# Exidekat/TransformerUpscaler

Hardware: AMD Instinct MI355X
Metric: images/sec, FastTransformer 2x 720p->1080p inference (higher is better)
Workload: dtype bf16

## Files before the change

transformerupscaler_amd/csrc/conv3x3_c64.hip:

```cpp
#include "conv_pingpong.h"
#include <stdlib.h>

namespace {

constexpr int TH = 8, TW = 32;
constexpr int in_tile_bytes(int ks) { return (TH + ks - 1) * (TW + ks - 1) * 128; }

enum { OUT_NHWC_BF16 = 0, OUT_PLANAR_F32 = 1 };

template <int CT, int OUT_MODE, int KS>
__global__ __launch_bounds__(256, (CT <= 4 && KS == 3) ? 2 : 1) void conv3x3_c64_kernel(
    const bf16_t* __restrict__ x, const bf16_t* __restrict__ wp, const float* __restrict__ bias,
    const bf16_t* __restrict__ add, const bf16_t* __restrict__ mask,
    void* __restrict__ out, int H, int W, int ntiles, int r, int cout_valid, int relu,
    int tilesX, int tilesY, int in_r)
{
    constexpr int PADK = KS / 2, HALO_W = TW + KS - 1, HALO_H = TH + KS - 1, NPIX_HALO = HALO_H * HALO_W;
    constexpr int NTAPS = KS * KS;
    extern __shared__ __attribute__((aligned(16))) char smem[];
    char* in_lds = smem;
    char* w_lds = smem + in_tile_bytes(KS);
    constexpr int WROWS = CT * 16;
    constexpr int WSLAB = WROWS * 128;
    constexpr int WCH = WROWS * 8;
    constexpr int WREGS = (WCH + 255) / 256;

    const int tid = threadIdx.x, lane = tid & 63, wave = tid >> 6;
    const int g = lane >> 4, p = lane & 15;
    int bid = blockIdx.x;
    const int tx = bid % tilesX; bid /= tilesX;
    const int ty = bid % tilesY;
    const int b = bid / tilesY;
    const int ty0 = ty * TH, tx0 = tx * TW;

    const int nci = in_r * in_r;
    const int Hin = H * in_r, Win = W * in_r;
    const bf16_t* xb = x + (size_t)b * Hin * Win * 64;
    constexpr int NSI = (NPIX_HALO * 8 + 255) / 256;
    auto stage_input = [&](int ci) {
        const int si = ci / in_r, sj = ci - si * in_r;
        u32x4 v[NSI];
        auto pos = [&](int idx, int& q, int& c, size_t& off) -> bool {
            q = idx >> 3; c = idx & 7;
            const int yy = q / HALO_W, xx = q - yy * HALO_W;
            const int iy = ty0 - PADK + yy, ix = tx0 - PADK + xx;
            const bool ok = idx < NPIX_HALO * 8 && iy >= 0 && iy < H && ix >= 0 && ix < W;
            off = ok ? ((size_t)(iy * in_r + si) * Win + (ix * in_r + sj)) * 64 + c * 8 : 0;
            return ok;
        };
#pragma unroll
        for (int k = 0; k < NSI; ++k) {
            int q, c; size_t off;
            pos(tid + k * 256, q, c, off);
            v[k] = *reinterpret_cast<const u32x4*>(xb + off);
        }
#pragma unroll
        for (int k = 0; k < NSI; ++k) {
            const int idx = tid + k * 256;
            int q, c; size_t off;
            const bool ok = pos(idx, q, c, off);
            if (idx < NPIX_HALO * 8) *reinterpret_cast<u32x4*>(in_lds + swz128(q, c)) = ok ? v[k] : u32x4{0u, 0u, 0u, 0u};
        }
    };
    stage_input(0);

    u32x4 wreg[WREGS];
    auto wload = [&](int it) {
#pragma unroll
        for (int u = 0; u < WREGS; ++u) {
            const int idx = tid + u * 256;
            if (idx < WCH) wreg[u] = *reinterpret_cast<const u32x4*>(wp + (size_t)it * WROWS * 64 + idx * 8);
        }
    };
    auto wstore = [&](int buf) {
#pragma unroll
        for (int u = 0; u < WREGS; ++u) {
            const int idx = tid + u * 256;
            if (idx < WCH) *reinterpret_cast<u32x4*>(w_lds + buf * WSLAB + swz128(idx >> 3, idx & 7)) = wreg[u];
        }
    };

    int qb[4];
#pragma unroll
    for (int pg = 0; pg < 4; ++pg) qb[pg] = (2 * wave + (pg >> 1)) * HALO_W + (pg & 1) * 16 + p;

    f32x4 acc[4][CT], bv[CT];
    const int total = ntiles * nci * NTAPS;
    wload(0);
    wstore(0);
    __syncthreads();

    for (int it = 0; it < total; ++it) {
        const int tap = it % NTAPS, chunk_it = it / NTAPS;
        const int ci = chunk_it % nci, nt = chunk_it / nci;
        const int buf = it & 1;
        if (tap == 0 && it > 0 && nci > 1) {
            stage_input(ci);
            __syncthreads();
        }
        if (it + 1 < total) wload(it + 1);
        if (tap == 0 && ci == 0) {
#pragma unroll
            for (int pg = 0; pg < 4; ++pg)
#pragma unroll
                for (int ct = 0; ct < CT; ++ct) acc[pg][ct] = f32x4{0.f, 0.f, 0.f, 0.f};
#pragma unroll
            for (int ct = 0; ct < CT; ++ct) {
                bv[ct] = f32x4{0.f, 0.f, 0.f, 0.f};
                if (bias) {
                    if constexpr (OUT_MODE == OUT_NHWC_BF16) bv[ct] = *reinterpret_cast<const f32x4*>(bias + nt * 64 + g * 16 + ct * 4);
                    else {
#pragma unroll
                        for (int e = 0; e < 4; ++e) { const int co = 16 * ct + 4 * g + e; bv[ct][e] = co < cout_valid ? bias[co] : 0.f; }
                    }
                }
            }
        }
        const int dy = tap / KS, dx = tap - dy * KS;
        const int qoff = dy * HALO_W + dx;
        const char* wb = w_lds + buf * WSLAB;
#pragma unroll
        for (int kh = 0; kh < 2; ++kh) {
            const int chunk = kh * 4 + g;
            bf16x8 pf[4], wf[CT];
#pragma unroll
            for (int pg = 0; pg < 4; ++pg)
                pf[pg] = *reinterpret_cast<const bf16x8*>(in_lds + swz128(qb[pg] + qoff, chunk));
#pragma unroll
            for (int ct = 0; ct < CT; ++ct)
                wf[ct] = *reinterpret_cast<const bf16x8*>(wb + swz128(ct * 16 + p, chunk));
#pragma unroll
            for (int pg = 0; pg < 4; ++pg)
#pragma unroll
                for (int ct = 0; ct < CT; ++ct) acc[pg][ct] = mfma16x16x32(wf[ct], pf[pg], acc[pg][ct]);
        }
        if (it + 1 < total) wstore(buf ^ 1);
        __syncthreads();

        if (tap == NTAPS - 1 && ci == nci - 1) {
#pragma unroll
            for (int pg = 0; pg < 4; ++pg) {
                const int oy = ty0 + 2 * wave + (pg >> 1);
                const int ox = tx0 + (pg & 1) * 16 + p;
                if (oy >= H || ox >= W) continue;
                if constexpr (OUT_MODE == OUT_NHWC_BF16) {
                    const int si = nt / r, sj = nt - si * r;
                    const int Hr = H * r, Wr = W * r;
                    bf16_t* o = reinterpret_cast<bf16_t*>(out) +
                                (((size_t)b * Hr + (oy * r + si)) * Wr + (ox * r + sj)) * 64 + g * 16;
                    uint32_t pk[8];
                    const size_t eoff = (((size_t)b * Hr + (oy * r + si)) * Wr + (ox * r + sj)) * 64 + g * 16;
                    uint32_t aw[8], mw[8];
                    if (add) {
                        const u32x4 a0 = *reinterpret_cast<const u32x4*>(add + eoff), a1 = *reinterpret_cast<const u32x4*>(add + eoff + 8);
#pragma unroll
                        for (int q = 0; q < 4; ++q) { aw[q] = a0[q]; aw[4 + q] = a1[q]; }
                    }
                    if (mask) {
                        const u32x4 m0 = *reinterpret_cast<const u32x4*>(mask + eoff), m1 = *reinterpret_cast<const u32x4*>(mask + eoff + 8);
#pragma unroll
                        for (int q = 0; q < 4; ++q) { mw[q] = m0[q]; mw[4 + q] = m1[q]; }
                    }
#pragma unroll
                    for (int ct = 0; ct < CT; ++ct) {
                        float v[4];
#pragma unroll
                        for (int e = 0; e < 4; ++e) {
                            v[e] = acc[pg][ct][e];
                            v[e] += bv[ct][e];
                            if (relu) v[e] = fmaxf(v[e], 0.f);
                            const int wi = (ct * 4 + e) >> 1;
                            if (add) v[e] += __builtin_bit_cast(float, (e & 1) ? (aw[wi] & 0xffff0000u) : (aw[wi] << 16));
                            if (mask) {
                                const float mv = __builtin_bit_cast(float, (e & 1) ? (mw[wi] & 0xffff0000u) : (mw[wi] << 16));
                                if (!(mv > 0.f)) v[e] = 0.f;
                            }
                        }
                        pk[ct * 2 + 0] = pack_bf16x2(v[0], v[1]);
                        pk[ct * 2 + 1] = pack_bf16x2(v[2], v[3]);
                    }
                    if constexpr (CT == 4) {
                        *reinterpret_cast<u32x4*>(o) = u32x4{pk[0], pk[1], pk[2], pk[3]};
                        *reinterpret_cast<u32x4*>(o + 8) = u32x4{pk[4], pk[5], pk[6], pk[7]};
                    }
                } else {
                    float* o = reinterpret_cast<float*>(out);
                    const int rr = r * r, cimg = cout_valid / rr, Hr = H * r, Wr = W * r;
#pragma unroll
                    for (int ct = 0; ct < CT; ++ct)
#pragma unroll
                        for (int e = 0; e < 4; ++e) {
                            const int co = 16 * ct + 4 * g + e;
                            if (co < cout_valid) {
                                float v = acc[pg][ct][e];
                                v += bv[ct][e];
                                if (relu) v = fmaxf(v, 0.f);
                                const int c = co / rr, sp = co - c * rr;
                                const int si = sp / r, sj = sp - si * r;
                                o[(((size_t)b * cimg + c) * Hr + (oy * r + si)) * Wr + (ox * r + sj)] = v;
                            }
                        }
                }
            }
        }
    }
}



__device__ unsigned long long tup_conv_stamps[2][16][5];

template <int CT, int OUT_MODE, int KS>
__global__ __launch_bounds__(512, 2) void conv_c64_persistent_kernel(
    const bf16_t* __restrict__ x, const bf16_t* __restrict__ wp, const float* __restrict__ bias,
    const bf16_t* __restrict__ add, const bf16_t* __restrict__ mask,
    void* __restrict__ out, int B, int H, int W, int ntiles, int r, int cout_valid, int relu,
    int tilesX, int tilesY, int stamps)
{
    constexpr int PADK = KS / 2, HALO_W = TW + KS - 1, HALO_H = TH + KS - 1, NPIX_HALO = HALO_H * HALO_W;
    constexpr int NTAPS = KS * KS;
    constexpr int IN_BYTES = NPIX_HALO * 128;
    constexpr int WROWS = CT * 16, WSLAB = WROWS * 128;
    extern __shared__ __attribute__((aligned(16))) char smem[];
    char* w_lds = smem;
    char* in_lds = smem + NTAPS * WSLAB;

    const int grp = __builtin_amdgcn_readfirstlane((int)(threadIdx.x >> 8));
    const int tid = threadIdx.x & 255, lane = tid & 63, wave = tid >> 6;
    const int g = lane >> 4, p = lane & 15;
    const int total_tiles = tilesX * tilesY * B;
    char* my_in = in_lds + grp * IN_BYTES;

    const HaloDma<HALO_H, HALO_W, PADK> dma(W, tid);
    auto prefetch_tile = [&](const TC& c) { dma.prefetch(x, c.b, c.ty * TH, c.tx * TW, H, W, my_in, tup_zero_line); };

    uint32_t poff[NTAPS][2];
    pixel_frag_offsets<KS, HALO_W>(poff, my_in, wave, g, p);
    const uint32_t wbase0 = weight_frag_base(w_lds, g, p);

    f32x4 acc[4][CT];
    float* bias_lds = reinterpret_cast<float*>(in_lds + 2 * IN_BYTES);
    const uint32_t bias_addr = lds_addr(bias_lds) + (uint32_t)(g * CT * 16);

    auto store_tile = [&](const TC& c, int nt) {
        const int tx = c.tx, ty = c.ty, b = c.b;
#pragma unroll
        for (int pg = 0; pg < 4; ++pg) {
            const int oy = ty * TH + 2 * wave + (pg >> 1);
            const int ox = tx * TW + (pg & 1) * 16 + p;
            const bool ok = oy < H && ox < W;
            if constexpr (OUT_MODE == OUT_NHWC_BF16) {
                const int si = nt / r, sj = nt - si * r;
                const int Hr = H * r, Wr = W * r;
                const size_t eoff = (((size_t)b * Hr + (oy * r + si)) * Wr + (ox * r + sj)) * 64 + g * 16;
                uint32_t pk[8], aw[8], mw[8];
                if (add && ok) {
                    const u32x4 a0 = *reinterpret_cast<const u32x4*>(add + eoff), a1 = *reinterpret_cast<const u32x4*>(add + eoff + 8);
#pragma unroll
                    for (int q = 0; q < 4; ++q) { aw[q] = a0[q]; aw[4 + q] = a1[q]; }
                }
                if (mask && ok) {
                    const u32x4 m0 = *reinterpret_cast<const u32x4*>(mask + eoff), m1 = *reinterpret_cast<const u32x4*>(mask + eoff + 8);
#pragma unroll
                    for (int q = 0; q < 4; ++q) { mw[q] = m0[q]; mw[4 + q] = m1[q]; }
                }
                if (!add && !mask) {
                    typedef short s16x2 __attribute__((ext_vector_type(2)));
#pragma unroll
                    for (int ct = 0; ct < CT; ++ct) {
                        pk[ct * 2 + 0] = pack_bf16x2(acc[pg][ct][0], acc[pg][ct][1]);
                        pk[ct * 2 + 1] = pack_bf16x2(acc[pg][ct][2], acc[pg][ct][3]);
                    }
                    if (relu) {
#pragma unroll
                        for (int q = 0; q < 2 * CT; ++q)
                            pk[q] = __builtin_bit_cast(uint32_t, __builtin_elementwise_max(__builtin_bit_cast(s16x2, pk[q]), s16x2{0, 0}));
                    }
                } else
#pragma unroll
                for (int ct = 0; ct < CT; ++ct) {
                    float v[4];
#pragma unroll
                    for (int e = 0; e < 4; ++e) {
                        v[e] = acc[pg][ct][e];
                        if (relu) v[e] = fmaxf(v[e], 0.f);
                        const int wi = (ct * 4 + e) >> 1;
                        if (add && ok) v[e] += __builtin_bit_cast(float, (e & 1) ? (aw[wi] & 0xffff0000u) : (aw[wi] << 16));
                        if (mask && ok) {
                            const float mv = __builtin_bit_cast(float, (e & 1) ? (mw[wi] & 0xffff0000u) : (mw[wi] << 16));
                            if (!(mv > 0.f)) v[e] = 0.f;
                        }
                    }
                    pk[ct * 2 + 0] = pack_bf16x2(v[0], v[1]);
                    pk[ct * 2 + 1] = pack_bf16x2(v[2], v[3]);
                }
                if constexpr (CT == 4) {
                    bf16_t* o = ok ? reinterpret_cast<bf16_t*>(out) + eoff : reinterpret_cast<bf16_t*>(tup_store_sink) + lane * 16;
                    *reinterpret_cast<u32x4*>(o) = u32x4{pk[0], pk[1], pk[2], pk[3]};
                    *reinterpret_cast<u32x4*>(o + 8) = u32x4{pk[4], pk[5], pk[6], pk[7]};
                }
            } else {
                if (!ok) continue;
                float* o = reinterpret_cast<float*>(out);
                const int rr = r * r, cimg = cout_valid / rr, Hr = H * r, Wr = W * r;
                if (CT == 1 && r == 2) {
                    if (g < cimg) {
                        float v[4];
#pragma unroll
                        for (int e = 0; e < 4; ++e) v[e] = relu ? fmaxf(acc[pg][0][e], 0.f) : acc[pg][0][e];
                        float* base = o + (((size_t)b * cimg + g) * Hr + oy * 2) * Wr + ox * 2;
                        *reinterpret_cast<f32x2*>(base) = f32x2{v[0], v[1]};
                        *reinterpret_cast<f32x2*>(base + Wr) = f32x2{v[2], v[3]};
                    }
                    continue;
                }
#pragma unroll
                for (int ct = 0; ct < CT; ++ct)
#pragma unroll
                    for (int e = 0; e < 4; ++e) {
                        const int co = 16 * ct + 4 * g + e;
                        if (co < cout_valid) {
                            float v = acc[pg][ct][e];
                            if (relu) v = fmaxf(v, 0.f);
                            const int c = co / rr, sp = co - c * rr;
                            const int si = sp / r, sj = sp - si * r;
                            o[(((size_t)b * cimg + c) * Hr + (oy * r + si)) * Wr + (ox * r + sj)] = v;
                        }
                    }
            }
        }
    };

    const TileWalk walk(total_tiles, tilesX, tilesY, grp, !(stamps & 2));
    const int my_count = walk.my_count, nphases = walk.nphases;
    const TC c_first = walk.first;

    for (int nt = 0; nt < ntiles; ++nt) {
        stage_weights<CT, NTAPS>(w_lds, wp + (size_t)nt * NTAPS * WROWS * 64);
        stage_bias<CT, OUT_MODE != OUT_NHWC_BF16>(bias_lds, bias, nt, cout_valid);
        if (grp == 0 && my_count > 0) prefetch_tile(c_first);
        __syncthreads();
        TC c_done = c_first, c_next = c_first;
        if (grp == 0) walk.advance(c_next);

        const bool st_on = (stamps & 1) && blockIdx.x == 100 && (threadIdx.x & 255) == 0 && nt == 0;
        auto stamp = [&](int ph, int i) { if (st_on && ph < 16) tup_conv_stamps[grp][ph][i] = __builtin_amdgcn_s_memtime(); };
        for (int ph = 0; ph < nphases; ++ph) {
            const int k = ph >> 1;
            stamp(ph, 0);
            if ((ph & 1) == grp) {
                if (k < my_count && !(stamps & 16)) k_loop<CT, NTAPS>(acc, poff, wbase0, bias_addr);
                stamp(ph, 1);
            } else {
                const int done = grp == 0 ? k : k - 1;
                const int nxt = done + 1;
                if (nxt < my_count && !(stamps & 8)) prefetch_tile(c_next);
                stamp(ph, 1);
                if (done >= 0 && done < my_count && !(stamps & 4)) {
                    store_tile(c_done, nt);
                    stamp(ph, 2);
                    if constexpr (OUT_MODE == OUT_NHWC_BF16 && CT == 4) asm volatile("s_waitcnt vmcnt(8)" ::: "memory");
                    else asm volatile("s_waitcnt vmcnt(0)" ::: "memory");
                } else {
                    asm volatile("s_waitcnt vmcnt(0)" ::: "memory");
                }
                c_done = c_next;
                walk.advance(c_next);
            }
            asm volatile("s_waitcnt lgkmcnt(0)" ::: "memory");
            stamp(ph, 3);
            __builtin_amdgcn_s_barrier();
            stamp(ph, 4);
        }
        asm volatile("s_waitcnt vmcnt(0)" ::: "memory");
        __syncthreads();
    }
}

template <int CT, int OUT_MODE, int KS>
int launch_persistent(const void* x, const void* wp, const float* bias, const void* add, const void* mask, void* out,
                      int B, int H, int W, int ntiles, int r, int cout_valid, int relu, hipStream_t s)
{
    constexpr int NPIX_HALO = (TH + KS - 1) * (TW + KS - 1);
    constexpr size_t lds = (size_t)KS * KS * CT * 16 * 128 + 2 * (size_t)NPIX_HALO * 128 + 256;
    static_assert(lds <= 163840, "LDS budget");
    TUP_SET_DYN_LDS((conv_c64_persistent_kernel<CT, OUT_MODE, KS>), lds);
    const int tilesX = (W + TW - 1) / TW, tilesY = (H + TH - 1) / TH;
    const long long nt = (long long)tilesX * tilesY * B;
    if (nt > 0x7fffffffLL) return (int)hipErrorInvalidValue;
    const int grid = (int)(nt < 256 ? nt : 256);
#ifdef TUP_DIAG
    static const int conv_stamps_on = (getenv("TUP_CONV_STAMPS") ? 1 : 0) | (getenv("TUP_CONV_NO_XCD_BANDS") ? 2 : 0) |
                                      (getenv("TUP_CONV_ABLATE") ? (atoi(getenv("TUP_CONV_ABLATE")) & 28) : 0);
#else
    constexpr int conv_stamps_on = 0;
#endif
    conv_c64_persistent_kernel<CT, OUT_MODE, KS><<<dim3(grid), dim3(512), lds, s>>>(
        (const bf16_t*)x, (const bf16_t*)wp, bias, (const bf16_t*)add, (const bf16_t*)mask, out, B, H, W, ntiles, r,
        cout_valid, relu, tilesX, tilesY, conv_stamps_on);
    TUP_CHECK_LAUNCH();
    return 0;
}

constexpr int R5_TW = 28, R5_HW = 32, R5_HH = TH + 4, R5_NPIX = R5_HH * R5_HW, R5_IN_BYTES = R5_NPIX * 128;
constexpr int R5_W_BYTES = 5 * 64 * 128;

__global__ __launch_bounds__(512, 2) void bra_rows_persistent_kernel(
    const bf16_t* __restrict__ x, const bf16_t* __restrict__ wp, const float* __restrict__ bias,
    float* __restrict__ out, int B, int H, int W, int relu, int tilesX, int tilesY, int ablate)
{
    extern __shared__ __attribute__((aligned(16))) char smem[];
    char* w_lds = smem;
    char* in_lds = smem + R5_W_BYTES;
    const int grp = __builtin_amdgcn_readfirstlane((int)(threadIdx.x >> 8));
    const int tid = threadIdx.x & 255, lane = tid & 63, wave = tid >> 6;
    const int g = lane >> 4, p = lane & 15;
    const int total_tiles = tilesX * tilesY * B;
    char* my_in = in_lds + grp * R5_IN_BYTES;

    using Dma = HaloDma<R5_HH, R5_HW, 2>;
    static_assert(!Dma::LAST_PARTIAL && Dma::NPIECE == 12, "12 whole DMA pieces");
    const Dma dma(W, tid);
    auto prefetch_tile = [&](const TC& c) { dma.prefetch(x, c.b, c.ty * TH, c.tx * R5_TW, H, W, my_in, tup_zero_line); };

    for (int idx = threadIdx.x; idx < 5 * 64 * 8; idx += 512) {
        const int row = idx >> 3, c = idx & 7;
        const int dy = row >> 6, t = (row >> 4) & 3, r16 = row & 15;
        const int gg = r16 >> 2, sl = t * 4 + (r16 & 3);
        u32x4 v = u32x4{0u, 0u, 0u, 0u};
        if (sl < 15) {
            const int ch = sl / 5, dx = sl - ch * 5;
            v = *reinterpret_cast<const u32x4*>(wp + ((size_t)((dy * 5 + dx) * 16 + ch * 4 + gg)) * 64 + c * 8);
        }
        *reinterpret_cast<u32x4*>(w_lds + swz128(row, c)) = v;
    }
    float bch[3];
#pragma unroll
    for (int ch = 0; ch < 3; ++ch) bch[ch] = bias ? bias[ch * 4 + g] : 0.f;

    const uint32_t pbase = lds_addr(my_in) + (uint32_t)(2 * wave * R5_HW * 128) + (uint32_t)swz128(p, g);
    const uint32_t wbase = lds_addr(w_lds) + (uint32_t)swz128(p, g);

    f32x4 acc[2][2][4];
    auto compute_tile = [&]() {
        constexpr int NSTEPS = 10;
        bf16x8 pf[3][4], wf[3][4];
        auto load_frag = [&](int step, int slot, int j) {
            const int dy = step >> 1;
            if (j < 4) {
                const int off = ((j >> 1) + dy) * (R5_HW * 128) + (j & 1) * 2048;
                pf[slot][j] = (step & 1) ? lds_read_b128_asm_off_x64(pbase, off) : lds_read_b128_asm_off(pbase, off);
            } else {
                const int off = dy * 8192 + (j - 4) * 2048;
                wf[slot][j - 4] = (step & 1) ? lds_read_b128_asm_off_x64(wbase, off) : lds_read_b128_asm_off(wbase, off);
            }
        };
#pragma unroll
        for (int j = 0; j < 8; ++j) load_frag(0, 0, j);
#pragma unroll
        for (int j = 0; j < 8; ++j) load_frag(1, 1, j);
#pragma unroll
        for (int rw = 0; rw < 2; ++rw)
#pragma unroll
            for (int cg = 0; cg < 2; ++cg)
#pragma unroll
                for (int t = 0; t < 4; ++t) acc[rw][cg][t] = f32x4{0.f, 0.f, 0.f, 0.f};
#pragma unroll
        for (int step = 0; step < NSTEPS; ++step) {
            const int cur = step % 3;
            if (step + 1 < NSTEPS) lds_wait<8>(); else lds_wait<0>();
            __builtin_amdgcn_sched_barrier(0);
#pragma unroll
            for (int j = 0; j < 8; ++j) {
                if (step + 2 < NSTEPS) load_frag(step + 2, (step + 2) % 3, j);
                const int i = j >> 1, t0 = (j & 1) * 2;
                acc[i >> 1][i & 1][t0] = mfma16x16x32(wf[cur][t0], pf[cur][i], acc[i >> 1][i & 1][t0]);
                acc[i >> 1][i & 1][t0 + 1] = mfma16x16x32(wf[cur][t0 + 1], pf[cur][i], acc[i >> 1][i & 1][t0 + 1]);
                __builtin_amdgcn_sched_barrier(0);
            }
        }
    };

    auto store_tile = [&](const TC& c) {
        const int tx = c.tx, ty = c.ty, b = c.b;
        const int Wr = W * 2, si = g >> 1, sj = g & 1;
        const int plane = 4 * H * W;
        float* outb = out + (size_t)b * 3 * plane;
#pragma unroll
        for (int rw = 0; rw < 2; ++rw) {
            const int oy = ty * TH + 2 * wave + rw;
#pragma unroll
            for (int cg = 0; cg < 2; ++cg) {
                const int xo = cg * 16 + p, ox = tx * R5_TW + xo;
                const bool ok = oy < H && ox < W && xo < R5_TW;
                float* o = ok ? outb + ((oy * 2 + si) * Wr + (ox * 2 + sj)) : reinterpret_cast<float*>(tup_store_sink) + lane;
                const int pstep = ok ? plane : 0;
#pragma unroll
                for (int ch = 0; ch < 3; ++ch) {
                    auto part = [&](int c2, int dx) { const int sl = ch * 5 + dx; return acc[rw][c2][sl >> 2][sl & 3]; };
                    float v = part(cg, 0) + bch[ch];
                    TUP_ADD_DPP(v, part(cg, 1), "row_shl:1"); TUP_ADD_DPP(v, part(cg, 2), "row_shl:2");
                    TUP_ADD_DPP(v, part(cg, 3), "row_shl:3"); TUP_ADD_DPP(v, part(cg, 4), "row_shl:4");
                    if (cg == 0) {
                        TUP_ADD_DPP(v, part(1, 1), "row_shr:15"); TUP_ADD_DPP(v, part(1, 2), "row_shr:14");
                        TUP_ADD_DPP(v, part(1, 3), "row_shr:13"); TUP_ADD_DPP(v, part(1, 4), "row_shr:12");
                    }
                    if (relu) v = fmaxf(v, 0.f);
                    o[ch * pstep] = v;
                }
            }
        }
    };

    const TileWalk walk(total_tiles, tilesX, tilesY, grp, !(ablate & 8));
    const int my_count = walk.my_count, nphases = walk.nphases;
    TC c_done = walk.first, c_next = walk.first;
    if (grp == 0 && my_count > 0) prefetch_tile(c_next);
    if (grp == 0) walk.advance(c_next);
    __syncthreads();
    for (int ph = 0; ph < nphases; ++ph) {
        const int k = ph >> 1;
        if ((ph & 1) == grp) {
            if (k < my_count && !(ablate & 1)) compute_tile();
        } else {
            const int done = grp == 0 ? k : k - 1;
            const int nxt = done + 1;
            if (nxt < my_count && !(ablate & 4)) prefetch_tile(c_next);
            if (done >= 0 && done < my_count && !(ablate & 2)) {
                store_tile(c_done);
                asm volatile("s_waitcnt vmcnt(12)" ::: "memory");
            } else {
                asm volatile("s_waitcnt vmcnt(0)" ::: "memory");
            }
            c_done = c_next;
            walk.advance(c_next);
        }
        asm volatile("s_waitcnt lgkmcnt(0)" ::: "memory");
        __builtin_amdgcn_s_barrier();
    }
    asm volatile("s_waitcnt vmcnt(0)" ::: "memory");
}

int launch_bra_rows(const void* x, const void* wp, const float* bias, float* out, int B, int H, int W, int relu, hipStream_t s)
{
    constexpr size_t lds = (size_t)R5_W_BYTES + 2 * (size_t)R5_IN_BYTES;
    static_assert(lds <= 163840, "LDS budget");
    TUP_SET_DYN_LDS(bra_rows_persistent_kernel, lds);
    const int tilesX = (W + R5_TW - 1) / R5_TW, tilesY = (H + TH - 1) / TH;
    const long long nt = (long long)tilesX * tilesY * B;
    if (nt > 0x7fffffffLL) return (int)hipErrorInvalidValue;
    const int grid = (int)(nt < 256 ? nt : 256);
    static const int ablate = TUP_ENV_INT("TUP_BRA_ABLATE", 0);
    bra_rows_persistent_kernel<<<dim3(grid), dim3(512), lds, s>>>((const bf16_t*)x, (const bf16_t*)wp, bias, out, B, H, W, relu, tilesX, tilesY, ablate);
    TUP_CHECK_LAUNCH();
    return 0;
}

constexpr int T3_TW = 28, T3_HW = 32, T3_HH = TH + 2, T3_NPIX = T3_HH * T3_HW, T3_IN_BYTES = T3_NPIX * 128;

__global__ __launch_bounds__(256, 3) void conv3_thin_rows_kernel(
    const bf16_t* __restrict__ x, const bf16_t* __restrict__ wp, const float* __restrict__ bias,
    float* __restrict__ out, int B, int H, int W, int cout, int relu, int tilesX, int tilesY)
{
    extern __shared__ __attribute__((aligned(16))) char smem[];
    const int tid = threadIdx.x, lane = tid & 63, wave = tid >> 6;
    const int g = lane >> 4, p = lane & 15;
    const int total_tiles = tilesX * tilesY * B;

    using Dma = HaloDma<T3_HH, T3_HW, 1>;
    static_assert(!Dma::LAST_PARTIAL && Dma::NPIECE == 10, "10 whole DMA pieces");
    const Dma dma(W, tid);
    auto prefetch_tile = [&](int tile) {
        int t = tile;
        const int tx = t % tilesX; t /= tilesX;
        const int ty = t % tilesY;
        const int b = t / tilesY;
        dma.prefetch(x, b, ty * TH, tx * T3_TW, H, W, smem, tup_zero_line);
    };

    bf16x8 wfr[3][2];
    {
        const int c = p >> 2, dx = p & 3;
        const bool live = dx < 3 && c < cout;
#pragma unroll
        for (int dy = 0; dy < 3; ++dy)
#pragma unroll
            for (int kh = 0; kh < 2; ++kh) {
                u32x4 v = u32x4{0u, 0u, 0u, 0u};
                if (live) v = *reinterpret_cast<const u32x4*>(wp + ((size_t)((dy * 3 + dx) * 16 + c)) * 64 + kh * 32 + g * 8);
                wfr[dy][kh] = __builtin_bit_cast(bf16x8, v);
            }
    }
    const float bv = (bias && g < cout) ? bias[g] : 0.f;
    const uint32_t pbase = lds_addr(smem) + (uint32_t)(2 * wave * T3_HW * 128) + (uint32_t)swz128(p, g);

    f32x4 acc[2][2];
    auto compute_tile = [&]() {
        bf16x8 pf[6][4];
#pragma unroll
        for (int st = 0; st < 6; ++st)
#pragma unroll
            for (int i = 0; i < 4; ++i) {
                const int off = ((i >> 1) + (st >> 1)) * (T3_HW * 128) + (i & 1) * 2048;
                pf[st][i] = (st & 1) ? lds_read_b128_asm_off_x64(pbase, off) : lds_read_b128_asm_off(pbase, off);
            }
#pragma unroll
        for (int i = 0; i < 4; ++i) acc[i >> 1][i & 1] = f32x4{0.f, 0.f, 0.f, 0.f};
#pragma unroll
        for (int st = 0; st < 6; ++st) {
            if (st == 0) lds_wait<15>(); else if (st == 1) lds_wait<15>(); else if (st == 2) lds_wait<12>();
            else if (st == 3) lds_wait<8>(); else if (st == 4) lds_wait<4>(); else lds_wait<0>();
            __builtin_amdgcn_sched_barrier(0);
#pragma unroll
            for (int i = 0; i < 4; ++i) acc[i >> 1][i & 1] = mfma16x16x32(wfr[st >> 1][st & 1], pf[st][i], acc[i >> 1][i & 1]);
            __builtin_amdgcn_sched_barrier(0);
        }
    };
    auto store_tile = [&](int tile) {
        int t = tile;
        const int tx = t % tilesX; t /= tilesX;
        const int ty = t % tilesY;
        const int b = t / tilesY;
        float* outb = out + ((size_t)b * cout + g) * H * W;
#pragma unroll
        for (int rw = 0; rw < 2; ++rw) {
            const int oy = ty * TH + 2 * wave + rw;
#pragma unroll
            for (int cg = 0; cg < 2; ++cg) {
                const int xo = cg * 16 + p, ox = tx * T3_TW + xo;
                float v = acc[rw][cg][0] + bv;
                TUP_ADD_DPP(v, acc[rw][cg][1], "row_shl:1"); TUP_ADD_DPP(v, acc[rw][cg][2], "row_shl:2");
                if (cg == 0) { TUP_ADD_DPP(v, acc[rw][1][1], "row_shr:15"); TUP_ADD_DPP(v, acc[rw][1][2], "row_shr:14"); }
                if (relu) v = fmaxf(v, 0.f);
                if (g < cout && oy < H && ox < W && xo < T3_TW) outb[(size_t)oy * W + ox] = v;
            }
        }
    };

    int first, stride, limit;
    xcd_band(total_tiles, true, first, stride, limit);
    if (first < limit) prefetch_tile(first);
    for (int tile = first; tile < limit; tile += stride) {
        asm volatile("s_waitcnt vmcnt(0)" ::: "memory");
        __builtin_amdgcn_s_barrier();
        compute_tile();
        asm volatile("s_waitcnt lgkmcnt(0)" ::: "memory");
        __builtin_amdgcn_s_barrier();
        if (tile + stride < limit) prefetch_tile(tile + stride);
        store_tile(tile);
    }
}

int launch_thin_rows(const void* x, const void* wp, const float* bias, float* out, int B, int H, int W, int cout, int relu, hipStream_t s)
{
    const int tilesX = (W + T3_TW - 1) / T3_TW, tilesY = (H + TH - 1) / TH;
    const long long nt = (long long)tilesX * tilesY * B;
    if (nt > 0x7fffffffLL) return (int)hipErrorInvalidValue;
    const int grid = (int)(nt < 768 ? nt : 768);
    conv3_thin_rows_kernel<<<dim3(grid), dim3(256), T3_IN_BYTES, s>>>((const bf16_t*)x, (const bf16_t*)wp, bias, out, B, H, W, cout, relu, tilesX, tilesY);
    TUP_CHECK_LAUNCH();
    return 0;
}

__global__ __launch_bounds__(256) void conv5x5_border_fix_kernel(
    const bf16_t* __restrict__ x, const bf16_t* __restrict__ wv, const float* __restrict__ bv,
    float* __restrict__ out, int B, int H, int W, int r, int relu)
{
    const int lane = threadIdx.x & 63;
    const int Hs = H * r, Ws = W * r, rr = r * r, nout = 3 * rr;
    const int per_img = 2 * Ws + 2 * (Hs - 2);
    const long long gid = (long long)blockIdx.x * 4 + (threadIdx.x >> 6);
    if (gid >= (long long)per_img * B) return;
    const int b = (int)(gid / per_img);
    int k = (int)(gid - (long long)b * per_img);
    int Y, X;
    if (k < Ws) { Y = 0; X = k; }
    else if (k < 2 * Ws) { Y = Hs - 1; X = k - Ws; }
    else { k -= 2 * Ws; Y = 1 + (k >> 1); X = (k & 1) ? Ws - 1 : 0; }
    const int rowmode = (Y == 0) ? 1 : (Y == Hs - 1 ? 2 : 0), colmode = (X == 0) ? 1 : (X == Ws - 1 ? 2 : 0);
    const int v = rowmode * 3 + colmode;
    const int y = Y / r, si = Y - y * r, xx0 = X / r, sj = X - xx0 * r;
    const int sp = si * r + sj;
    float a0 = 0.f, a1 = 0.f, a2 = 0.f;
    const int t8 = lane >> 3, c8 = lane & 7;
    u32x4 fx[4], fw[4][3];
    bool use[4];
#pragma unroll
    for (int rd = 0; rd < 4; ++rd) {
        const int tap = rd * 8 + t8;
        const int ty = tap / 5, tx = tap - ty * 5;
        const int iy = y + ty - 2, ix = xx0 + tx - 2;
        use[rd] = tap < 25 && iy >= 0 && iy < H && ix >= 0 && ix < W;
        const int tapc = tap < 25 ? tap : 24, iyc = min(max(iy, 0), H - 1), ixc = min(max(ix, 0), W - 1);
        fx[rd] = *reinterpret_cast<const u32x4*>(x + (((size_t)b * H + iyc) * W + ixc) * 64 + c8 * 8);
        const bf16_t* wb = wv + (((size_t)v * nout) * 25 + tapc) * 64 + c8 * 8;
#pragma unroll
        for (int c = 0; c < 3; ++c) fw[rd][c] = *reinterpret_cast<const u32x4*>(wb + (size_t)(c * rr + sp) * 25 * 64);
    }
#pragma unroll
    for (int rd = 0; rd < 4; ++rd) {
        if (!use[rd]) continue;
#pragma unroll
        for (int q = 0; q < 4; ++q) {
            const float xl = __builtin_bit_cast(float, fx[rd][q] << 16), xh = __builtin_bit_cast(float, fx[rd][q] & 0xffff0000u);
            a0 = fmaf(xl, __builtin_bit_cast(float, fw[rd][0][q] << 16), a0); a0 = fmaf(xh, __builtin_bit_cast(float, fw[rd][0][q] & 0xffff0000u), a0);
            a1 = fmaf(xl, __builtin_bit_cast(float, fw[rd][1][q] << 16), a1); a1 = fmaf(xh, __builtin_bit_cast(float, fw[rd][1][q] & 0xffff0000u), a1);
            a2 = fmaf(xl, __builtin_bit_cast(float, fw[rd][2][q] << 16), a2); a2 = fmaf(xh, __builtin_bit_cast(float, fw[rd][2][q] & 0xffff0000u), a2);
        }
    }
#pragma unroll
    for (int o = 32; o >= 1; o >>= 1) { a0 += __shfl_xor(a0, o); a1 += __shfl_xor(a1, o); a2 += __shfl_xor(a2, o); }
    if (lane < 3) {
        float val = (lane == 0 ? a0 : (lane == 1 ? a1 : a2)) + bv[v * nout + lane * rr + sp];
        if (relu) val = fmaxf(val, 0.f);
        out[(((size_t)b * 3 + lane) * Hs + Y) * Ws + X] = val;
    }
}

}

extern "C" int tup_conv3x3_c64_fwd(const void* x, const void* wp, const float* bias, const void* add,
                                   const void* mask, void* out, int B, int H, int W, int ntiles, int r,
                                   int cout_valid, int relu, int out_mode, int in_r, void* stream)
{
    if (B <= 0 || H <= 0 || W <= 0) return 0;
    if (in_r < 1 || in_r > 6) return (int)hipErrorInvalidValue;
    const int tilesX = (W + TW - 1) / TW, tilesY = (H + TH - 1) / TH;
    const long long nblk = (long long)tilesX * tilesY * B;
    if (nblk > 0x7fffffffLL) return (int)hipErrorInvalidValue;
    hipStream_t s = reinterpret_cast<hipStream_t>(stream);
    static const bool use_persistent = !TUP_ENV_FLAG("TUP_CONV_NONPERSISTENT");
    if (in_r == 1 && use_persistent) {
        if (out_mode == OUT_NHWC_BF16) {
            if (ntiles != r * r || r < 1) return (int)hipErrorInvalidValue;
            return launch_persistent<4, OUT_NHWC_BF16, 3>(x, wp, bias, add, mask, out, B, H, W, ntiles, r, 64, relu, s);
        }
        if (out_mode == OUT_PLANAR_F32) {
            if (ntiles != 1 || r != 1 || cout_valid < 1 || cout_valid > 16 || add || mask) return (int)hipErrorInvalidValue;
            static const bool thin_pingpong = TUP_ENV_FLAG("TUP_THIN_PINGPONG");
            if (cout_valid <= 4 && !thin_pingpong) return launch_thin_rows(x, wp, bias, (float*)out, B, H, W, cout_valid, relu, s);
            return launch_persistent<1, OUT_PLANAR_F32, 3>(x, wp, bias, nullptr, nullptr, out, B, H, W, 1, 1, cout_valid, relu, s);
        }
        return (int)hipErrorInvalidValue;
    }
    if (out_mode == OUT_NHWC_BF16) {
        if (ntiles != r * r || r < 1) return (int)hipErrorInvalidValue;
        const size_t lds = in_tile_bytes(3) + 2 * 64 * 128;
        conv3x3_c64_kernel<4, OUT_NHWC_BF16, 3><<<dim3((unsigned)nblk), dim3(256), lds, s>>>(
            (const bf16_t*)x, (const bf16_t*)wp, bias, (const bf16_t*)add, (const bf16_t*)mask, out, H, W, ntiles, r,
            64, relu, tilesX, tilesY, in_r);
    } else if (out_mode == OUT_PLANAR_F32) {
        if (ntiles != 1 || r != 1 || cout_valid < 1 || cout_valid > 16 || add || mask) return (int)hipErrorInvalidValue;
        const size_t lds = in_tile_bytes(3) + 2 * 16 * 128;
        conv3x3_c64_kernel<1, OUT_PLANAR_F32, 3><<<dim3((unsigned)nblk), dim3(256), lds, s>>>(
            (const bf16_t*)x, (const bf16_t*)wp, bias, nullptr, nullptr, out, H, W, 1, 1, cout_valid, relu, tilesX,
            tilesY, in_r);
    } else {
        return (int)hipErrorInvalidValue;
    }
    TUP_CHECK_LAUNCH();
    return 0;
}

extern "C" int tup_conv5x5_c64_planar_fwd(const void* x, const void* wp, const float* bias, const void* wv,
                                          const float* bv, float* out, int B, int H, int W, int r, int relu,
                                          void* stream)
{
    if (B <= 0 || H <= 0 || W <= 0) return 0;
    if (!(r == 2 || r == 3 || r == 6)) return (int)hipErrorInvalidValue;
    const int tilesX = (W + TW - 1) / TW, tilesY = (H + TH - 1) / TH;
    const long long nblk = (long long)tilesX * tilesY * B;
    if (nblk > 0x7fffffffLL) return (int)hipErrorInvalidValue;
    hipStream_t s = reinterpret_cast<hipStream_t>(stream);
    const int nout = 3 * r * r;
    static const bool use_persistent5 = !TUP_ENV_FLAG("TUP_CONV_NONPERSISTENT");
    static const bool use_taps25 = TUP_ENV_FLAG("TUP_BRA_TAPS25");
    if (r == 2 && use_persistent5) {
        int e = use_taps25 ? launch_persistent<1, OUT_PLANAR_F32, 5>(x, wp, bias, nullptr, nullptr, out, B, H, W, 1, r, nout, relu, s)
                           : launch_bra_rows(x, wp, bias, out, B, H, W, relu, s);
        if (e) return e;
    } else if (r == 2) {
        conv3x3_c64_kernel<1, OUT_PLANAR_F32, 5><<<dim3((unsigned)nblk), dim3(256), in_tile_bytes(5) + 2 * 16 * 128, s>>>(
            (const bf16_t*)x, (const bf16_t*)wp, bias, nullptr, nullptr, out, H, W, 1, r, nout, relu, tilesX, tilesY, 1);
    } else if (r == 3) {
        const size_t lds = in_tile_bytes(5) + 2 * 32 * 128;
        TUP_SET_DYN_LDS((conv3x3_c64_kernel<2, OUT_PLANAR_F32, 5>), lds);
        conv3x3_c64_kernel<2, OUT_PLANAR_F32, 5><<<dim3((unsigned)nblk), dim3(256), lds, s>>>(
            (const bf16_t*)x, (const bf16_t*)wp, bias, nullptr, nullptr, out, H, W, 1, r, nout, relu, tilesX, tilesY, 1);
    } else {
        const size_t lds = in_tile_bytes(5) + 2 * 112 * 128;
        TUP_SET_DYN_LDS((conv3x3_c64_kernel<7, OUT_PLANAR_F32, 5>), lds);
        conv3x3_c64_kernel<7, OUT_PLANAR_F32, 5><<<dim3((unsigned)nblk), dim3(256), lds, s>>>(
            (const bf16_t*)x, (const bf16_t*)wp, bias, nullptr, nullptr, out, H, W, 1, r, nout, relu, tilesX, tilesY, 1);
    }
    TUP_CHECK_LAUNCH();
    const long long nborder = (long long)B * (2LL * W * r + 2LL * (H * r - 2));
    conv5x5_border_fix_kernel<<<dim3((unsigned)((nborder + 3) / 4)), dim3(256), 0, s>>>(
        (const bf16_t*)x, (const bf16_t*)wv, bv, out, B, H, W, r, relu);
    TUP_CHECK_LAUNCH();
    return 0;
}

#ifdef TUP_DIAG
extern "C" int tup_debug_conv_stamps(unsigned long long* host_out)
{
    return (int)hipMemcpyFromSymbol(host_out, HIP_SYMBOL(tup_conv_stamps), sizeof(unsigned long long) * 2 * 16 * 5);
}
#endif
```

Measured before the change: 2616.

## Repack 5x5 pixel-shuffle weights to skip zero MFMA slabs and vectorize stores

Result: faster. 2659 (median of 6 runs) (+1.6%).

```diff
diff --git a/transformerupscaler_amd/csrc/conv3x3_c64.hip b/transformerupscaler_amd/csrc/conv3x3_c64.hip
--- a/transformerupscaler_amd/csrc/conv3x3_c64.hip
+++ b/transformerupscaler_amd/csrc/conv3x3_c64.hip
@@ -403,7 +403,10 @@
 }
 
 constexpr int R5_TW = 28, R5_HW = 32, R5_HH = TH + 4, R5_NPIX = R5_HH * R5_HW, R5_IN_BYTES = R5_NPIX * 128;
-constexpr int R5_W_BYTES = 5 * 64 * 128;
+constexpr int R5_NSLAB = 2 + 3 * 4 + 2, R5_W_BYTES = R5_NSLAB * 16 * 128;
+constexpr int r5_slab(int dy, int t) { return dy == 0 ? t : (dy == 4 ? 12 + t : 2 + (dy - 1) * 4 + t); }
+constexpr int r5_ntiles(int dy) { return (dy == 0 || dy == 4) ? 2 : 4; }
+constexpr int r5_tile0(int dy) { return dy == 4 ? 2 : 0; }
 
 __global__ __launch_bounds__(512, 2) void bra_rows_persistent_kernel(
     const bf16_t* __restrict__ x, const bf16_t* __restrict__ wp, const float* __restrict__ bias,
@@ -423,20 +426,19 @@
     const Dma dma(W, tid);
     auto prefetch_tile = [&](const TC& c) { dma.prefetch(x, c.b, c.ty * TH, c.tx * R5_TW, H, W, my_in, tup_zero_line); };
 
-    for (int idx = threadIdx.x; idx < 5 * 64 * 8; idx += 512) {
+    for (int idx = threadIdx.x; idx < R5_NSLAB * 16 * 8; idx += 512) {
         const int row = idx >> 3, c = idx & 7;
-        const int dy = row >> 6, t = (row >> 4) & 3, r16 = row & 15;
-        const int gg = r16 >> 2, sl = t * 4 + (r16 & 3);
+        const int slab = row >> 4, r16 = row & 15;
+        const int dy = slab < 2 ? 0 : (slab < 14 ? 1 + ((slab - 2) >> 2) : 4);
+        const int t = slab < 2 ? slab : (slab < 14 ? (slab - 2) & 3 : slab - 12);
+        const int ch = r16 >> 2, dx = (r16 & 3) + (t & 1);
         u32x4 v = u32x4{0u, 0u, 0u, 0u};
-        if (sl < 15) {
-            const int ch = sl / 5, dx = sl - ch * 5;
-            v = *reinterpret_cast<const u32x4*>(wp + ((size_t)((dy * 5 + dx) * 16 + ch * 4 + gg)) * 64 + c * 8);
-        }
+        if (ch < 3) v = *reinterpret_cast<const u32x4*>(wp + ((size_t)((dy * 5 + dx) * 16 + ch * 4 + t)) * 64 + c * 8);
         *reinterpret_cast<u32x4*>(w_lds + swz128(row, c)) = v;
     }
-    float bch[3];
-#pragma unroll
-    for (int ch = 0; ch < 3; ++ch) bch[ch] = bias ? bias[ch * 4 + g] : 0.f;
+    float bsp[4];
+#pragma unroll
+    for (int t = 0; t < 4; ++t) bsp[t] = (bias && g < 3) ? bias[g * 4 + t] : 0.f;
 
     const uint32_t pbase = lds_addr(my_in) + (uint32_t)(2 * wave * R5_HW * 128) + (uint32_t)swz128(p, g);
     const uint32_t wbase = lds_addr(w_lds) + (uint32_t)swz128(p, g);
@@ -451,14 +453,15 @@
                 const int off = ((j >> 1) + dy) * (R5_HW * 128) + (j & 1) * 2048;
                 pf[slot][j] = (step & 1) ? lds_read_b128_asm_off_x64(pbase, off) : lds_read_b128_asm_off(pbase, off);
             } else {
-                const int off = dy * 8192 + (j - 4) * 2048;
+                const int off = r5_slab(dy, r5_tile0(dy) + j - 4) * 2048;
                 wf[slot][j - 4] = (step & 1) ? lds_read_b128_asm_off_x64(wbase, off) : lds_read_b128_asm_off(wbase, off);
             }
         };
-#pragma unroll
-        for (int j = 0; j < 8; ++j) load_frag(0, 0, j);
-#pragma unroll
-        for (int j = 0; j < 8; ++j) load_frag(1, 1, j);
+        auto nfrag = [](int step) { return 4 + r5_ntiles(step >> 1); };
+#pragma unroll
+        for (int j = 0; j < nfrag(0); ++j) load_frag(0, 0, j);
+#pragma unroll
+        for (int j = 0; j < nfrag(1); ++j) load_frag(1, 1, j);
 #pragma unroll
         for (int rw = 0; rw < 2; ++rw)
 #pragma unroll
@@ -467,46 +470,55 @@
                 for (int t = 0; t < 4; ++t) acc[rw][cg][t] = f32x4{0.f, 0.f, 0.f, 0.f};
 #pragma unroll
         for (int step = 0; step < NSTEPS; ++step) {
-            const int cur = step % 3;
-            if (step + 1 < NSTEPS) lds_wait<8>(); else lds_wait<0>();
+            const int cur = step % 3, dy = step >> 1;
+            const int npair = 2 * r5_ntiles(dy), t00 = r5_tile0(dy);
+            const int nld = step + 2 < NSTEPS ? nfrag(step + 2) : 0;
+            if (step + 1 >= NSTEPS) lds_wait<0>(); else if (nfrag(step + 1) == 8) lds_wait<8>(); else lds_wait<6>();
             __builtin_amdgcn_sched_barrier(0);
 #pragma unroll
-            for (int j = 0; j < 8; ++j) {
-                if (step + 2 < NSTEPS) load_frag(step + 2, (step + 2) % 3, j);
-                const int i = j >> 1, t0 = (j & 1) * 2;
-                acc[i >> 1][i & 1][t0] = mfma16x16x32(wf[cur][t0], pf[cur][i], acc[i >> 1][i & 1][t0]);
-                acc[i >> 1][i & 1][t0 + 1] = mfma16x16x32(wf[cur][t0 + 1], pf[cur][i], acc[i >> 1][i & 1][t0 + 1]);
+            for (int j = 0; j < npair; ++j) {
+#pragma unroll
+                for (int l = j * nld / npair; l < (j + 1) * nld / npair; ++l) load_frag(step + 2, (step + 2) % 3, l);
+                const int i = npair == 8 ? (j >> 1) : j, w0 = npair == 8 ? (j & 1) * 2 : 0, t0 = t00 + w0;
+                acc[i >> 1][i & 1][t0] = mfma16x16x32(wf[cur][w0], pf[cur][i], acc[i >> 1][i & 1][t0]);
+                acc[i >> 1][i & 1][t0 + 1] = mfma16x16x32(wf[cur][w0 + 1], pf[cur][i], acc[i >> 1][i & 1][t0 + 1]);
                 __builtin_amdgcn_sched_barrier(0);
             }
         }
     };
 
-    auto store_tile = [&](const TC& c) {
+    auto store_tile = [&](const TC& c, auto RELU) {
         const int tx = c.tx, ty = c.ty, b = c.b;
-        const int Wr = W * 2, si = g >> 1, sj = g & 1;
-        const int plane = 4 * H * W;
-        float* outb = out + (size_t)b * 3 * plane;
+        const int Wr = W * 2;
+        float* outb = out + ((size_t)b * 3 + g) * 4 * H * W;
+        if (g >= 3) return;
 #pragma unroll
         for (int rw = 0; rw < 2; ++rw) {
             const int oy = ty * TH + 2 * wave + rw;
 #pragma unroll
             for (int cg = 0; cg < 2; ++cg) {
                 const int xo = cg * 16 + p, ox = tx * R5_TW + xo;
-                const bool ok = oy < H && ox < W && xo < R5_TW;
-                float* o = ok ? outb + ((oy * 2 + si) * Wr + (ox * 2 + sj)) : reinterpret_cast<float*>(tup_store_sink) + lane;
-                const int pstep = ok ? plane : 0;
-#pragma unroll
-                for (int ch = 0; ch < 3; ++ch) {
-                    auto part = [&](int c2, int dx) { const int sl = ch * 5 + dx; return acc[rw][c2][sl >> 2][sl & 3]; };
-                    float v = part(cg, 0) + bch[ch];
-                    TUP_ADD_DPP(v, part(cg, 1), "row_shl:1"); TUP_ADD_DPP(v, part(cg, 2), "row_shl:2");
-                    TUP_ADD_DPP(v, part(cg, 3), "row_shl:3"); TUP_ADD_DPP(v, part(cg, 4), "row_shl:4");
+                const bool ok = oy < H && ox < W;
+                float* o = ok ? outb + (oy * 2 * Wr + ox * 2) : reinterpret_cast<float*>(tup_store_sink) + 2 * lane;
+                const int rstep = ok ? Wr : 0;
+#pragma unroll
+                for (int si = 0; si < 2; ++si) {
+                    const f32x4 &a0 = acc[rw][cg][si * 2], &a1 = acc[rw][cg][si * 2 + 1];
+                    float v0 = a0[0] + bsp[si * 2], v1 = bsp[si * 2 + 1];
+                    TUP_ADD_DPP(v0, a0[1], "row_shl:1"); TUP_ADD_DPP(v0, a0[2], "row_shl:2"); TUP_ADD_DPP(v0, a0[3], "row_shl:3");
+                    TUP_ADD_DPP(v1, a1[0], "row_shl:1"); TUP_ADD_DPP(v1, a1[1], "row_shl:2");
+                    TUP_ADD_DPP(v1, a1[2], "row_shl:3"); TUP_ADD_DPP(v1, a1[3], "row_shl:4");
                     if (cg == 0) {
-                        TUP_ADD_DPP(v, part(1, 1), "row_shr:15"); TUP_ADD_DPP(v, part(1, 2), "row_shr:14");
-                        TUP_ADD_DPP(v, part(1, 3), "row_shr:13"); TUP_ADD_DPP(v, part(1, 4), "row_shr:12");
-                    }
-                    if (relu) v = fmaxf(v, 0.f);
-                    o[ch * pstep] = v;
+                        const f32x4 &n0 = acc[rw][1][si * 2], &n1 = acc[rw][1][si * 2 + 1];
+                        TUP_ADD_DPP(v0, n0[1], "row_shr:15"); TUP_ADD_DPP(v0, n0[2], "row_shr:14"); TUP_ADD_DPP(v0, n0[3], "row_shr:13");
+                        TUP_ADD_DPP(v1, n1[0], "row_shr:15"); TUP_ADD_DPP(v1, n1[1], "row_shr:14");
+                        TUP_ADD_DPP(v1, n1[2], "row_shr:13"); TUP_ADD_DPP(v1, n1[3], "row_shr:12");
+                    }
+                    if constexpr (decltype(RELU)::value) {
+                        asm("v_max_f32 %0, 0, %0" : "+v"(v0));
+                        asm("v_max_f32 %0, 0, %0" : "+v"(v1));
+                    }
+                    if (cg == 0 || p < R5_TW - 16) *reinterpret_cast<f32x2*>(o + si * rstep) = f32x2{v0, v1};
                 }
             }
         }
@@ -527,8 +539,8 @@
             const int nxt = done + 1;
             if (nxt < my_count && !(ablate & 4)) prefetch_tile(c_next);
             if (done >= 0 && done < my_count && !(ablate & 2)) {
-                store_tile(c_done);
-                asm volatile("s_waitcnt vmcnt(12)" ::: "memory");
+                if (relu) store_tile(c_done, std::true_type{}); else store_tile(c_done, std::false_type{});
+                asm volatile("s_waitcnt vmcnt(8)" ::: "memory");
             } else {
                 asm volatile("s_waitcnt vmcnt(0)" ::: "memory");
             }
@@ -548,7 +560,7 @@
     TUP_SET_DYN_LDS(bra_rows_persistent_kernel, lds);
     const int tilesX = (W + R5_TW - 1) / R5_TW, tilesY = (H + TH - 1) / TH;
     const long long nt = (long long)tilesX * tilesY * B;
-    if (nt > 0x7fffffffLL) return (int)hipErrorInvalidValue;
+    if (nt > 0x7fffffffLL || (reinterpret_cast<uintptr_t>(out) & 7)) return (int)hipErrorInvalidValue;
     const int grid = (int)(nt < 256 ? nt : 256);
     static const int ablate = TUP_ENV_INT("TUP_BRA_ABLATE", 0);
     bra_rows_persistent_kernel<<<dim3(grid), dim3(512), lds, s>>>((const bf16_t*)x, (const bf16_t*)wp, bias, out, B, H, W, relu, tilesX, tilesY, ablate);
@@ -662,17 +674,17 @@
     return 0;
 }
 
+template <int R>
 __global__ __launch_bounds__(256) void conv5x5_border_fix_kernel(
     const bf16_t* __restrict__ x, const bf16_t* __restrict__ wv, const float* __restrict__ bv,
-    float* __restrict__ out, int B, int H, int W, int r, int relu)
-{
+    float* __restrict__ out, int B, int H, int W, int relu)
+{
+    constexpr int r = R, rr = r * r, nout = 3 * rr;
     const int lane = threadIdx.x & 63;
-    const int Hs = H * r, Ws = W * r, rr = r * r, nout = 3 * rr;
+    const int Hs = H * r, Ws = W * r;
     const int per_img = 2 * Ws + 2 * (Hs - 2);
-    const long long gid = (long long)blockIdx.x * 4 + (threadIdx.x >> 6);
-    if (gid >= (long long)per_img * B) return;
-    const int b = (int)(gid / per_img);
-    int k = (int)(gid - (long long)b * per_img);
+    int k = (int)blockIdx.x * 4 + __builtin_amdgcn_readfirstlane((int)(threadIdx.x >> 6));
+    if (k >= per_img) return;
     int Y, X;
     if (k < Ws) { Y = 0; X = k; }
     else if (k < 2 * Ws) { Y = Hs - 1; X = k - Ws; }
@@ -681,39 +693,39 @@
     const int v = rowmode * 3 + colmode;
     const int y = Y / r, si = Y - y * r, xx0 = X / r, sj = X - xx0 * r;
     const int sp = si * r + sj;
-    float a0 = 0.f, a1 = 0.f, a2 = 0.f;
-    const int t8 = lane >> 3, c8 = lane & 7;
-    u32x4 fx[4], fw[4][3];
-    bool use[4];
-#pragma unroll
-    for (int rd = 0; rd < 4; ++rd) {
-        const int tap = rd * 8 + t8;
-        const int ty = tap / 5, tx = tap - ty * 5;
-        const int iy = y + ty - 2, ix = xx0 + tx - 2;
-        use[rd] = tap < 25 && iy >= 0 && iy < H && ix >= 0 && ix < W;
-        const int tapc = tap < 25 ? tap : 24, iyc = min(max(iy, 0), H - 1), ixc = min(max(ix, 0), W - 1);
-        fx[rd] = *reinterpret_cast<const u32x4*>(x + (((size_t)b * H + iyc) * W + ixc) * 64 + c8 * 8);
+    for (int b = blockIdx.y; b < B; b += gridDim.y) {
+        float a0 = 0.f, a1 = 0.f, a2 = 0.f;
+        const int ylo = (si + (rowmode == 1 ? 1 : 0) - 1 + r) / r, yhi = (si + (rowmode == 2 ? 1 : 2) - 1 + r) / r + 2;
+        const int xlo = (sj + (colmode == 1 ? 1 : 0) - 1 + r) / r, xhi = (sj + (colmode == 2 ? 1 : 2) - 1 + r) / r + 2;
+        const int ty0 = max(ylo, 2 - y), tx0 = max(xlo, 2 - xx0);
+        const int ny = min(yhi, H + 1 - y) - ty0 + 1, nx = min(xhi, W + 1 - xx0) - tx0 + 1;
+        const int t8 = lane >> 3, c8 = lane & 7;
+        const int rcp = nx == 1 ? 32 : (nx == 2 ? 16 : (nx == 3 ? 11 : 8));
+        const int qy = (t8 * rcp) >> 5, ty = ty0 + qy, tx = tx0 + t8 - qy * nx;
+        const bool use = t8 < ny * nx;
+        const int tapc = use ? ty * 5 + tx : 12;
+        const int iyc = use ? y + ty - 2 : y, ixc = use ? xx0 + tx - 2 : xx0;
+        const u32x4 fx = *reinterpret_cast<const u32x4*>(x + (((size_t)b * H + iyc) * W + ixc) * 64 + c8 * 8);
         const bf16_t* wb = wv + (((size_t)v * nout) * 25 + tapc) * 64 + c8 * 8;
-#pragma unroll
-        for (int c = 0; c < 3; ++c) fw[rd][c] = *reinterpret_cast<const u32x4*>(wb + (size_t)(c * rr + sp) * 25 * 64);
-    }
-#pragma unroll
-    for (int rd = 0; rd < 4; ++rd) {
-        if (!use[rd]) continue;
-#pragma unroll
-        for (int q = 0; q < 4; ++q) {
-            const float xl = __builtin_bit_cast(float, fx[rd][q] << 16), xh = __builtin_bit_cast(float, fx[rd][q] & 0xffff0000u);
-            a0 = fmaf(xl, __builtin_bit_cast(float, fw[rd][0][q] << 16), a0); a0 = fmaf(xh, __builtin_bit_cast(float, fw[rd][0][q] & 0xffff0000u), a0);
-            a1 = fmaf(xl, __builtin_bit_cast(float, fw[rd][1][q] << 16), a1); a1 = fmaf(xh, __builtin_bit_cast(float, fw[rd][1][q] & 0xffff0000u), a1);
-            a2 = fmaf(xl, __builtin_bit_cast(float, fw[rd][2][q] << 16), a2); a2 = fmaf(xh, __builtin_bit_cast(float, fw[rd][2][q] & 0xffff0000u), a2);
-        }
-    }
-#pragma unroll
-    for (int o = 32; o >= 1; o >>= 1) { a0 += __shfl_xor(a0, o); a1 += __shfl_xor(a1, o); a2 += __shfl_xor(a2, o); }
-    if (lane < 3) {
-        float val = (lane == 0 ? a0 : (lane == 1 ? a1 : a2)) + bv[v * nout + lane * rr + sp];
-        if (relu) val = fmaxf(val, 0.f);
-        out[(((size_t)b * 3 + lane) * Hs + Y) * Ws + X] = val;
+        u32x4 fw[3];
+#pragma unroll
+        for (int c = 0; c < 3; ++c) fw[c] = *reinterpret_cast<const u32x4*>(wb + (size_t)(c * rr + sp) * 25 * 64);
+        if (use) {
+#pragma unroll
+            for (int q = 0; q < 4; ++q) {
+                const float xl = __builtin_bit_cast(float, fx[q] << 16), xh = __builtin_bit_cast(float, fx[q] & 0xffff0000u);
+                a0 = fmaf(xl, __builtin_bit_cast(float, fw[0][q] << 16), a0); a0 = fmaf(xh, __builtin_bit_cast(float, fw[0][q] & 0xffff0000u), a0);
+                a1 = fmaf(xl, __builtin_bit_cast(float, fw[1][q] << 16), a1); a1 = fmaf(xh, __builtin_bit_cast(float, fw[1][q] & 0xffff0000u), a1);
+                a2 = fmaf(xl, __builtin_bit_cast(float, fw[2][q] << 16), a2); a2 = fmaf(xh, __builtin_bit_cast(float, fw[2][q] & 0xffff0000u), a2);
+            }
+        }
+#pragma unroll
+        for (int o = 32; o >= 1; o >>= 1) { a0 += __shfl_xor(a0, o); a1 += __shfl_xor(a1, o); a2 += __shfl_xor(a2, o); }
+        if (lane < 3) {
+            float val = (lane == 0 ? a0 : (lane == 1 ? a1 : a2)) + bv[v * nout + lane * rr + sp];
+            if (relu) val = fmaxf(val, 0.f);
+            out[(((size_t)b * 3 + lane) * Hs + Y) * Ws + X] = val;
+        }
     }
 }
 
@@ -794,9 +806,13 @@
             (const bf16_t*)x, (const bf16_t*)wp, bias, nullptr, nullptr, out, H, W, 1, r, nout, relu, tilesX, tilesY, 1);
     }
     TUP_CHECK_LAUNCH();
-    const long long nborder = (long long)B * (2LL * W * r + 2LL * (H * r - 2));
-    conv5x5_border_fix_kernel<<<dim3((unsigned)((nborder + 3) / 4)), dim3(256), 0, s>>>(
-        (const bf16_t*)x, (const bf16_t*)wv, bv, out, B, H, W, r, relu);
+    const long long per_img = 2LL * W * r + 2LL * (H * r - 2);
+    if (per_img > 0x7fffffffLL) return (int)hipErrorInvalidValue;
+    const dim3 ring_grid((unsigned)((per_img + 3) / 4), (unsigned)(B < 65535 ? B : 65535));
+    const bf16_t* xb = (const bf16_t*)x; const bf16_t* wvb = (const bf16_t*)wv;
+    if (r == 2) conv5x5_border_fix_kernel<2><<<ring_grid, dim3(256), 0, s>>>(xb, wvb, bv, out, B, H, W, relu);
+    else if (r == 3) conv5x5_border_fix_kernel<3><<<ring_grid, dim3(256), 0, s>>>(xb, wvb, bv, out, B, H, W, relu);
+    else conv5x5_border_fix_kernel<6><<<ring_grid, dim3(256), 0, s>>>(xb, wvb, bv, out, B, H, W, relu);
     TUP_CHECK_LAUNCH();
     return 0;
 }
```
